# OzAmram/CaloDiffusion

Measured on AMD Instinct MI355X. Metric: sampled showers/sec (Dataset-2, 400-step DDIM), higher is better.
Workload: dtype f32 (convs: fp32 operands as 2-term fp16 splits on the fp16 MFMA pipe, fp32 accumulate; attention/norms fp32)

## Files before the change

calodiffusion_amd/csrc/kernels_conv_transpose.hip:

```cpp
#include "conv_internal.h"
#include <algorithm>
#include <vector>

namespace cd {

static constexpr int LDS_VOX_PAD = 4;

struct ConvTArgs {
  const float* in;
  int cin;
  const float* wpk;
  const float* bias;
  float* out;
  int Din, Hin, Win, Do, Ho, Wo;
  int KZ, SZ;
  int cout, CTtot;
  int TZ, TH, nTZ, nTH;
  int Cw;
  int CS;
  const u32x4* wpk16;
  int* status;
  const unsigned* in_absmax;
  int tr_off = 0;
};

template <int CT>
__global__ void __launch_bounds__(256) conv_transpose_kernel(ConvTArgs a) {
  extern __shared__ __attribute__((aligned(16))) float lds[];
  const int tid = threadIdx.x, lane = tid & 63, wave = tid >> 6, nw = blockDim.x >> 6;
  int bid = blockIdx.x;
  const int thi = bid % a.nTH;
  bid /= a.nTH;
  const int tzi = bid % a.nTZ;
  const int b = bid / a.nTZ;
  const int a0 = tzi * a.TZ, b0 = thi * a.TH;
  const int PZ = a.TZ + 2, PH = a.TH + 2;
  const int tileVox = PZ * PH * a.Win;
  const int ZERO = tileVox * a.CS;
  const int half = lane >> 5, col = lane & 31;
  for (int i = tid; i < a.CS; i += blockDim.x) lds[ZERO + i] = 0.f;

  {
    const int c4 = a.cin >> 2;
    const int items = tileVox * c4;
    const float* src = a.in + (size_t)b * a.Din * a.Hin * a.Win * a.cin;
    for (int idx = tid; idx < items; idx += blockDim.x) {
      const int q = idx % c4, vox = idx / c4;
      const int iw = vox % a.Win;
      const int r = vox / a.Win;
      const int lh = r % PH, lz = r / PH;
      const int gz = a0 - 1 + lz;
      int gh = (b0 - 1 + lh) % a.Hin;
      if (gh < 0) gh += a.Hin;
      f32x4 val = {0.f, 0.f, 0.f, 0.f};
      if (gz >= 0 && gz < a.Din) val = *(const f32x4*)(src + ((size_t)(gz * a.Hin + gh) * a.Win + iw) * a.cin + q * 4);
      *(f32x4*)(lds + vox * a.CS + q * 4) = val;
    }
  }
  __syncthreads();

  const int ncls = a.SZ * 4;
  const int njt = (a.TZ * a.TH * a.Cw + 31) / 32;
  const int nchunk = a.cin >> 5;
  const int T = a.KZ * 16;
  float* outb = a.out + (size_t)b * a.Do * a.Ho * a.Wo * a.cout;

  for (int job = wave; job < ncls * njt; job += nw) {
    const int cls = job / njt, jt = job % njt;
    const int pz = cls >> 2, ph = (cls >> 1) & 1, pw = cls & 1;
    const int v = jt * 32 + col;
    const int c = v % a.Cw;
    const int t = v / a.Cw;
    const int bb = t % a.TH, aa = t / a.TH;
    const int oz = a.SZ * (a0 + aa) + pz, oh = 2 * (b0 + bb) + ph, ow = 2 * c + pw;
    const bool valid = (aa < a.TZ) && (oz < a.Do) && (oh < a.Ho) && (ow < a.Wo);
    if (!__any(valid)) continue;
    const int ooff = valid ? ((oz * a.Ho + oh) * a.Wo + ow) * a.cout : -1;

    f32x16 acc[CT];
#pragma unroll
    for (int ct = 0; ct < CT; ++ct)
#pragma unroll
      for (int r = 0; r < 16; ++r) acc[ct][r] = 0.f;

    for (int kz = (pz + 1) % a.SZ; kz < a.KZ; kz += a.SZ) {
      const int lz = aa + (pz + 1 - kz) / a.SZ + 1;
      for (int kh = (ph + 3) & 1; kh < 4; kh += 2) {
        const int lh = bb + (ph + 3 - kh) / 2;
        for (int kw = (pw + 1) & 1; kw < 4; kw += 2) {
          const int iw = c + (pw + 1 - kw) / 2;
          const bool ok = valid && iw >= 0 && iw < a.Win;
          const int off = ok ? ((lz * PH + lh) * a.Win + iw) * a.CS + half * 16 : ZERO + half * 16;
          const int tap = (kz * 4 + kh) * 4 + kw;
          for (int chunk = 0; chunk < nchunk; ++chunk) {
            f32x4 av[4];
#pragma unroll
            for (int q = 0; q < 4; ++q) av[q] = *(const f32x4*)(lds + off + chunk * 32 + q * 4);
            const f32x4* wq = (const f32x4*)a.wpk + ((size_t)(chunk * T + tap) * a.CTtot) * 256 + lane;
#pragma unroll
            for (int ct = 0; ct < CT; ++ct) {
              f32x4 bw[4];
#pragma unroll
              for (int q = 0; q < 4; ++q) bw[q] = wq[ct * 256 + q * 64];
#pragma unroll
              for (int q = 0; q < 4; ++q)
#pragma unroll
                for (int e = 0; e < 4; ++e) acc[ct] = MFMA32(av[q][e], bw[q][e], acc[ct]);
            }
          }
        }
      }
    }
#pragma unroll
    for (int r = 0; r < 16; ++r) {
      const int row = (r & 3) + 8 * (r >> 2) + 4 * half;
      const int off = __shfl(ooff, row, 64);
      if (off >= 0) {
#pragma unroll
        for (int ct = 0; ct < CT; ++ct) {
          const int co = ct * 32 + col;
          outb[off + co] = acc[ct][r] + (a.bias ? a.bias[co] : 0.f);
        }
      }
    }
  }
}

template <int CT>
__global__ void __launch_bounds__(256) conv_transpose_f16x2_kernel(ConvTArgs a) {
  extern __shared__ __attribute__((aligned(16))) float lds[];
  const int tid = threadIdx.x, lane = tid & 63, wave = tid >> 6, nw = blockDim.x >> 6;
  int bid = blockIdx.x;
  const int thi = bid % a.nTH;
  bid /= a.nTH;
  const int tzi = bid % a.nTZ;
  const int b = bid / a.nTZ;
  const int a0 = tzi * a.TZ, b0 = thi * a.TH;
  const int PZ = a.TZ + 2, PH = a.TH + 2;
  const int tileVox = PZ * PH * a.Win;
  const int ZERO = tileVox * a.CS;
  const int half = lane >> 5, col = lane & 31;
  for (int i = tid; i < a.CS; i += blockDim.x) lds[ZERO + i] = 0.f;

  float gscale = 1.f, ginv = 1.f;
  if (a.in_absmax) pow2_scale_for(*a.in_absmax, &gscale, &ginv);
  {
    const int c4 = a.cin >> 2;
    const float* src = a.in + (size_t)b * a.Din * a.Hin * a.Win * a.cin;
    float amax = 0.f;
    auto stage = [&](int vox, int q, int iw, int lh, int lz) {
      const int gz = a0 - 1 + lz;
      int gh = b0 - 1 + lh;
      gh = gh < 0 ? gh + a.Hin : gh;
      gh = gh >= a.Hin ? gh - a.Hin : gh;
      gh = gh >= a.Hin ? gh - a.Hin : gh;
      f32x4 val = {0.f, 0.f, 0.f, 0.f};
      if (gz >= 0 && gz < a.Din) val = *(const f32x4*)(src + ((size_t)(gz * a.Hin + gh) * a.Win + iw) * a.cin + q * 4);
      val *= gscale;
      amax = fmaxf(amax, fmaxf(fmaxf(fabsf(val[0]), fabsf(val[1])), fmaxf(fabsf(val[2]), fabsf(val[3]))));
      u32x2 t1, t2;
      split2(val, t1, t2);
      char* dst = (char*)(lds + vox * a.CS) + (q >> 2) * 64 + (q & 3) * 8;
      *(u32x2*)dst = t1;
      *(u32x2*)(dst + 32) = t2;
    };
    const int nthr = blockDim.x;
    if (nthr % c4 == 0) {
      const int q = tid % c4, vstep = nthr / c4;
      int vox = tid / c4;
      int iw = vox % a.Win, r = vox / a.Win;
      int lh = r % PH, lz = r / PH;
      const int dw = vstep % a.Win, dr = vstep / a.Win, dh = dr % PH, dz = dr / PH;
      for (; vox < tileVox; vox += vstep) {
        stage(vox, q, iw, lh, lz);
        iw += dw; lh += dh; lz += dz;
        if (iw >= a.Win) { iw -= a.Win; lh += 1; }
        if (lh >= PH) { lh -= PH; lz += 1; }
      }
    } else {
      const int items = tileVox * c4;
      for (int idx = tid; idx < items; idx += nthr) {
        const int q = idx % c4, vox = idx / c4;
        const int iw = vox % a.Win;
        const int r = vox / a.Win;
        stage(vox, q, iw, r % PH, r / PH);
      }
    }
    if (a.status && amax > 65504.f) atomicOr(a.status, 1);
  }
  __syncthreads();

  const int szs = a.SZ - 1;
  const int ncls = a.SZ * 4;
  const int njt = (a.TZ * a.TH * a.Cw + 31) / 32;
  const int nks = a.cin >> 4;
  const int T = a.KZ * 16;
  float* outb = a.out + (size_t)b * a.Do * a.Ho * a.Wo * a.cout;

  const bool tile_major = njt >= nw;
  for (int item = wave; item < (tile_major ? njt : ncls * njt); item += nw) {
    const int jt = tile_major ? item : item % njt;
    const int v = jt * 32 + col;
    const int c = v % a.Cw;
    const int t = v / a.Cw;
    const int bb = t % a.TH, aa = t / a.TH;
  for (int ci = 0; ci < (tile_major ? ncls : 1); ++ci) {
    const int cls = tile_major ? ci : item / njt;
    const int pz = cls >> 2, ph = (cls >> 1) & 1, pw = cls & 1;
    const int oz = ((a0 + aa) << szs) + pz, oh = 2 * (b0 + bb) + ph, ow = 2 * c + pw;
    const bool valid = (aa < a.TZ) && (oz < a.Do) && (oh < a.Ho) && (ow < a.Wo);
    if (!__any(valid)) continue;
    const int ooff = valid ? ((oz * a.Ho + oh) * a.Wo + ow) * a.cout : -1;

    f32x16 accA[CT], accB[CT];
#pragma unroll
    for (int ct = 0; ct < CT; ++ct)
#pragma unroll
      for (int r = 0; r < 16; ++r) { accA[ct][r] = 0.f; accB[ct][r] = 0.f; }

    const int kz0 = (pz + 1) & szs, kh0 = (ph + 3) & 1, kw0 = (pw + 1) & 1;
    const int nkz = (a.KZ - kz0 + a.SZ - 1) >> szs;
    const int nstage = nkz * 4 * nks;
    struct Stage {
      u32x4 x1, x2, w[CT][2];
    };
    int ti_n = 0, ks_n = 0, tap_n = 0;
    const char* rec_n = nullptr;
    auto setup = [&](int ti) {
      const int kz = kz0 + ((ti >> 2) << szs), kh = kh0 + ((ti >> 1) & 1) * 2, kw = kw0 + (ti & 1) * 2;
      const int lz = aa + ((pz + 1 - kz) >> szs) + 1;
      const int lh = bb + ((ph + 3 - kh) >> 1);
      const int iw = c + ((pw + 1 - kw) >> 1);
      const bool ok = valid && iw >= 0 && iw < a.Win;
      rec_n = (const char*)(lds + (ok ? ((lz * PH + lh) * a.Win + iw) * a.CS : ZERO)) + half * 16;
      tap_n = (kz * 4 + kh) * 4 + kw;
    };
    setup(0);
    auto fetch = [&](Stage& st) {
      st.x1 = *(const u32x4*)(rec_n + ks_n * 64);
      st.x2 = *(const u32x4*)(rec_n + ks_n * 64 + 32);
      const u32x4* wq = a.wpk16 + ((size_t)(ks_n * T + tap_n) * a.CTtot) * 128 + lane;
#pragma unroll
      for (int ct = 0; ct < CT; ++ct) {
        st.w[ct][0] = wq[ct * 128];
        st.w[ct][1] = wq[ct * 128 + 64];
      }
      if (ks_n + 1 < nks) ++ks_n;
      else if (ti_n + 1 < nkz * 4) { ks_n = 0; setup(++ti_n); }
    };
    auto mfmas = [&](const Stage& st) {
#pragma unroll
      for (int ct = 0; ct < CT; ++ct) {
        accA[ct] = MFMA_F16(st.x1, st.w[ct][0], accA[ct]);
        accB[ct] = MFMA_F16(st.x1, st.w[ct][1], accB[ct]);
        accB[ct] = MFMA_F16(st.x2, st.w[ct][0], accB[ct]);
      }
    };
    Stage s0, s1, s2, s3;
    fetch(s0);
    fetch(s1);
    fetch(s2);
    for (int j = 0; j < nstage; j += 4) {
      fetch(s3);
      __builtin_amdgcn_sched_barrier(0);
      mfmas(s0);
      __builtin_amdgcn_sched_barrier(0);
      fetch(s0);
      __builtin_amdgcn_sched_barrier(0);
      if (j + 1 < nstage) mfmas(s1);
      __builtin_amdgcn_sched_barrier(0);
      fetch(s1);
      __builtin_amdgcn_sched_barrier(0);
      if (j + 2 < nstage) mfmas(s2);
      __builtin_amdgcn_sched_barrier(0);
      fetch(s2);
      __builtin_amdgcn_sched_barrier(0);
      if (j + 3 < nstage) mfmas(s3);
    }
    float* tr = lds + a.tr_off + wave * (32 * 36);
#pragma unroll
    for (int ct = 0; ct < CT; ++ct) {
      const float bv = a.bias ? a.bias[ct * 32 + col] : 0.f;
#pragma unroll
      for (int r = 0; r < 16; ++r)
        tr[((r & 3) + 8 * (r >> 2) + 4 * half) * 36 + col] = (accA[ct][r] + accB[ct][r] * (1.f / 2048.f)) * ginv + bv;
      asm volatile("s_waitcnt lgkmcnt(0)" ::: "memory");
#pragma unroll
      for (int k = 0; k < 4; ++k) {
        const int row = 8 * k + (lane >> 3);
        const int off = __shfl(ooff, row, 64);
        const f32x4 q = *(const f32x4*)(tr + row * 36 + (lane & 7) * 4);
        if (off >= 0) *(f32x4*)(outb + off + ct * 32 + (lane & 7) * 4) = q;
      }
      asm volatile("s_waitcnt lgkmcnt(0)" ::: "memory");
    }
  }
  }
}

template <int CT>
static void launch_convT_inst(const ConvTArgs& a, dim3 grid, size_t lds, hipStream_t s) {
  static bool attr_set = false;
  if (!attr_set) {
    CD_HIP(hipFuncSetAttribute((const void*)conv_transpose_kernel<CT>, hipFuncAttributeMaxDynamicSharedMemorySize, 160 * 1024));
    CD_HIP(hipFuncSetAttribute((const void*)conv_transpose_f16x2_kernel<CT>, hipFuncAttributeMaxDynamicSharedMemorySize, 160 * 1024));
    attr_set = true;
  }
  if (a.wpk16) hipLaunchKernelGGL((conv_transpose_f16x2_kernel<CT>), grid, dim3(256), lds, s, a);
  else hipLaunchKernelGGL((conv_transpose_kernel<CT>), grid, dim3(256), lds, s, a);
  CD_HIP(hipGetLastError());
}

void launch_conv_transpose_mfma(const float* in, int cin, const float* wpk, const float* bias, float* out, int batch,
                                int cout, Dims3 din, Dims3 dout, int kz, int sz, hipStream_t s, const void* wpk_f16x2,
                                int* status, const unsigned* in_absmax) {
  CD_REQUIRE(cin % 32 == 0 && cout % 32 == 0, "conv_transpose: channels must be multiples of 32");
  CD_REQUIRE(sz == 1 || sz == 2, "conv_transpose: z stride must be 1 or 2");
  const bool full_range = conv_precision() != PREC_F16X2;
  ConvTArgs a;
  a.wpk16 = full_range ? nullptr : (const u32x4*)wpk_f16x2;
  a.status = status;
  a.in_absmax = in_absmax;
  a.in = in; a.cin = cin; a.wpk = wpk; a.bias = bias; a.out = out;
  a.Din = din.d; a.Hin = din.h; a.Win = din.w; a.Do = dout.d; a.Ho = dout.h; a.Wo = dout.w;
  a.KZ = kz; a.SZ = sz; a.cout = cout; a.CTtot = cout / 32;
  a.Cw = (dout.w + 1) / 2;
  a.CS = cin + LDS_VOX_PAD;
  const int Az = (dout.d + sz - 1) / sz, Bh = (dout.h + 1) / 2;
  struct TT { int tz, th; double score; };
  std::vector<TT> all;
  for (int TZ = 1; TZ <= Az; ++TZ)
    for (int TH = 1; TH <= Bh; ++TH) {
      const size_t lds = ((size_t)(TZ + 2) * (TH + 2) * din.w + 1) * a.CS * 4;
      if (lds > 140 * 1024) break;
      if (TH != Bh && (Bh + TH - 1) / TH == (Bh + TH) / (TH + 1)) continue;
      if (TZ != Az && (Az + TZ - 1) / TZ == (Az + TZ) / (TZ + 1)) continue;
      const long nblocks = (long)batch * ((Az + TZ - 1) / TZ) * ((Bh + TH - 1) / TH);
      const double ratio = (double)TZ * TH / ((double)(TZ + 2) * (TH + 2));
      const double fill = nblocks >= 512 ? 1.0 : (double)nblocks / 512.0;
      all.push_back({TZ, TH, ratio * fill});
    }
  CD_REQUIRE(!all.empty(), "conv_transpose: no tile fits in LDS");
  std::stable_sort(all.begin(), all.end(), [](const TT& x, const TT& y) { return x.score > y.score; });
  std::vector<TT> cand;
  for (size_t i = 0; i < all.size() && cand.size() < 8; ++i) cand.push_back(all[i]);
  for (size_t i = 8; i < all.size() && cand.size() < 14; i += (all.size() - 8) / 6 + 1) cand.push_back(all[i]);
  char cat[128];
  std::snprintf(cat, sizeof cat, "convT%dx4x4 C%d->%d @%dx%dx%d", kz, cin, cout, din.d, din.h, din.w);
  prof::Scope scope(cat, s, 2.0 * kz * 16 * cin * cout * (double)din.vox() * batch,
                    4.0 * batch * ((double)din.vox() * cin + (double)dout.vox() * cout));
  auto launch = [&](const TT& t) {
    ConvTArgs b = a;
    b.TZ = t.tz; b.TH = t.th;
    b.nTZ = (Az + b.TZ - 1) / b.TZ; b.nTH = (Bh + b.TH - 1) / b.TH;
    size_t lds = ((size_t)(b.TZ + 2) * (b.TH + 2) * din.w + 1) * b.CS * 4;
    if (b.wpk16) {
      lds = (lds + 15) & ~(size_t)15;
      b.tr_off = (int)(lds / 4);
      lds += 4 * 32 * 36 * 4;
    }
    dim3 grid((unsigned)(batch * b.nTZ * b.nTH));
    switch (b.CTtot) {
      case 1: launch_convT_inst<1>(b, grid, lds, s); break;
      case 2: launch_convT_inst<2>(b, grid, lds, s); break;
      case 3: launch_convT_inst<3>(b, grid, lds, s); break;
      case 4: launch_convT_inst<4>(b, grid, lds, s); break;
      default: CD_REQUIRE(false, "conv_transpose: more than 128 output channels unsupported");
    }
  };
  char key[192];
  std::snprintf(key, sizeof key, "%s k%d s%d b%d%s", cat, kz, sz, batch, a.wpk16 ? " f16x2" : "");
  const int pick = autotune(key, (int)cand.size(), [&](int i) { launch(cand[i]); }, s);
  launch(cand[pick < 0 ? 0 : pick]);
}

}
```

Measured before the change: 90.89.

## Add weight-resident transposed-conv kernel with software-pipelined LDS loads

Adds a weight-resident variant of the f16x2 transposed-conv kernel for cin==cout in {32,64}. Each wave keeps one output class/channel-tile's weights in registers and sweeps all spatial tiles, prefetching LDS fragments three steps ahead and overlapping the previous tile's epilogue with the current MFMAs. The input staging loop is also unrolled so several global loads are in flight at once. Autotune candidates now include resident tile shapes with their own scoring, and env overrides are added. The cost is much higher register pressure, which may lower occupancy.

After: 91.11 (median of 2 runs). About the same (+0.2%).

```diff
diff --git a/calodiffusion_amd/csrc/kernels_conv_transpose.hip b/calodiffusion_amd/csrc/kernels_conv_transpose.hip
--- a/calodiffusion_amd/csrc/kernels_conv_transpose.hip
+++ b/calodiffusion_amd/csrc/kernels_conv_transpose.hip
@@ -1,5 +1,6 @@
 #include "conv_internal.h"
 #include <algorithm>
+#include <cstring>
 #include <vector>
 
 namespace cd {
@@ -24,6 +25,129 @@
   int tr_off = 0;
 };
 
+template <int NTAP, int NKS>
+__device__ __forceinline__ void convt_resident_job(const ConvTArgs& a, const float* lds, float* tr, float* outb, int cls, int ct, int a0,
+                                                   int b0, int PH, int ZERO, int njt, float ginv, int lane) {
+  constexpr int NST = NTAP * NKS, PF = 3;
+  static_assert(NST > PF, "convt_resident_job: pipeline deeper than the job");
+  const int half = lane >> 5, col = lane & 31;
+  const int szs = a.SZ - 1;
+  const int pz = cls >> 2, ph = (cls >> 1) & 1, pw = cls & 1;
+  const int kz0 = (pz + 1) & szs, kh0 = (ph + 3) & 1, kw0 = (pw + 1) & 1;
+  const int T = a.KZ * 16;
+  u32x4 w[NST][2];
+  int dB[NTAP];
+#pragma unroll
+  for (int ti = 0; ti < NTAP; ++ti) {
+    const int kz = kz0 + ((ti >> 2) << szs), kh = kh0 + ((ti >> 1) & 1) * 2, kw = kw0 + (ti & 1) * 2;
+    const int tap = (kz * 4 + kh) * 4 + kw;
+    dB[ti] = (((((pz + 1 - kz) >> szs) * PH + ((ph + 3 - kh) >> 1)) * a.Win + ((pw + 1 - kw) >> 1)) * a.CS) * 4;
+#pragma unroll
+    for (int ks = 0; ks < NKS; ++ks) {
+      const u32x4* wq = a.wpk16 + ((size_t)(ks * T + tap) * a.CTtot + ct) * 128 + lane;
+      w[ti * NKS + ks][0] = wq[0];
+      w[ti * NKS + ks][1] = wq[64];
+    }
+  }
+  const int dw0 = (pw + 1 - kw0) >> 1;
+  const int zaddr = ZERO * 4 + half * 16;
+  const float bv = a.bias ? a.bias[ct * 32 + col] : 0.f;
+
+  int c = col % a.Cw, bb, aa;
+  {
+    const int t = col / a.Cw;
+    bb = t % a.TH;
+    aa = t / a.TH;
+  }
+  const int dc = 32 % a.Cw, dt = 32 / a.Cw, db = dt % a.TH, da = dt / a.TH;
+  struct Frag {
+    u32x4 x1, x2;
+  };
+  bool valid = false, ok0 = false, ok1 = false;
+  int ooff = -1, base = 0;
+  auto place = [&]() {
+    const int oz = ((a0 + aa) << szs) + pz, oh = 2 * (b0 + bb) + ph, ow = 2 * c + pw;
+    valid = (aa < a.TZ) && (oz < a.Do) && (oh < a.Ho) && (ow < a.Wo);
+    ooff = valid ? ((oz * a.Ho + oh) * a.Wo + ow) * a.cout : -1;
+    base = ((((aa + 1) * PH + bb) * a.Win + c) * a.CS) * 4 + half * 16;
+    const int iw0 = c + dw0;
+    ok0 = valid && iw0 >= 0 && iw0 < a.Win;
+    ok1 = valid && iw0 >= 1 && iw0 - 1 < a.Win;
+  };
+  auto load = [&](Frag& f, int j) {
+    const int ti = j / NKS, ks = j % NKS;
+    const char* rec = (const char*)lds + (((ti & 1) ? ok1 : ok0) ? base + dB[ti] : zaddr);
+    f.x1 = *(const u32x4*)(rec + ks * 64);
+    f.x2 = *(const u32x4*)(rec + ks * 64 + 32);
+  };
+  Frag pre[PF];
+  place();
+#pragma unroll
+  for (int j = 0; j < PF; ++j) load(pre[j], j);
+  int ooff_prev = -1;
+  auto epi_write = [&](const f32x16& pA, const f32x16& pB) {
+#pragma unroll
+    for (int r = 0; r < 16; ++r)
+      tr[((r & 3) + 8 * (r >> 2) + 4 * half) * 36 + col] = (pA[r] + pB[r] * (1.f / 2048.f)) * ginv + bv;
+  };
+  f32x4 oq[4];
+  int ooffq[4];
+  auto epi_read = [&]() {
+#pragma unroll
+    for (int k = 0; k < 4; ++k) {
+      const int row = 8 * k + (lane >> 3);
+      ooffq[k] = __shfl(ooff_prev, row, 64);
+      oq[k] = *(const f32x4*)(tr + row * 36 + (lane & 7) * 4);
+    }
+  };
+  auto epi_store = [&]() {
+#pragma unroll
+    for (int k = 0; k < 4; ++k)
+      if (ooffq[k] >= 0) *(f32x4*)(outb + ooffq[k] + ct * 32 + (lane & 7) * 4) = oq[k];
+  };
+  auto tile = [&](f32x16& accA, f32x16& accB, const f32x16& pA, const f32x16& pB) {
+#pragma unroll
+    for (int r = 0; r < 16; ++r) { accA[r] = 0.f; accB[r] = 0.f; }
+    Frag x[NST];
+#pragma unroll
+    for (int j = 0; j < PF; ++j) x[j] = pre[j];
+#pragma unroll
+    for (int j = 0; j < NST; ++j) {
+      if (j + PF < NST) load(x[j + PF], j + PF);
+      accA = MFMA_F16(x[j].x1, w[j][0], accA);
+      accB = MFMA_F16(x[j].x1, w[j][1], accB);
+      accB = MFMA_F16(x[j].x2, w[j][0], accB);
+      if (j == 0) epi_write(pA, pB);
+      if (j == 2) epi_read();
+      if (j == 5) epi_store();
+    }
+    ooff_prev = ooff;
+    c += dc; bb += db; aa += da;
+    if (c >= a.Cw) { c -= a.Cw; bb += 1; }
+    if (bb >= a.TH) { bb -= a.TH; aa += 1; }
+    place();
+#pragma unroll
+    for (int j = 0; j < PF; ++j) load(pre[j], j);
+  };
+  f32x16 a0A, a0B, a1A, a1B;
+#pragma unroll
+  for (int r = 0; r < 16; ++r) { a1A[r] = 0.f; a1B[r] = 0.f; }
+  int jt = 0;
+  for (; jt + 1 < njt; jt += 2) {
+    tile(a0A, a0B, a1A, a1B);
+    tile(a1A, a1B, a0A, a0B);
+  }
+  if (jt < njt) {
+    tile(a0A, a0B, a1A, a1B);
+    epi_write(a0A, a0B);
+  } else {
+    epi_write(a1A, a1B);
+  }
+  epi_read();
+  epi_store();
+  asm volatile("s_waitcnt lgkmcnt(0)" ::: "memory");
+}
+
 template <int CT>
 __global__ void __launch_bounds__(256) conv_transpose_kernel(ConvTArgs a) {
   extern __shared__ __attribute__((aligned(16))) float lds[];
@@ -126,7 +250,7 @@
   }
 }
 
-template <int CT>
+template <int CT, bool RES = false>
 __global__ void __launch_bounds__(256) conv_transpose_f16x2_kernel(ConvTArgs a) {
   extern __shared__ __attribute__((aligned(16))) float lds[];
   const int tid = threadIdx.x, lane = tid & 63, wave = tid >> 6, nw = blockDim.x >> 6;
@@ -148,14 +272,15 @@
     const int c4 = a.cin >> 2;
     const float* src = a.in + (size_t)b * a.Din * a.Hin * a.Win * a.cin;
     float amax = 0.f;
-    auto stage = [&](int vox, int q, int iw, int lh, int lz) {
+    auto src_off = [&](int iw, int lh, int lz) {
       const int gz = a0 - 1 + lz;
       int gh = b0 - 1 + lh;
       gh = gh < 0 ? gh + a.Hin : gh;
       gh = gh >= a.Hin ? gh - a.Hin : gh;
       gh = gh >= a.Hin ? gh - a.Hin : gh;
-      f32x4 val = {0.f, 0.f, 0.f, 0.f};
-      if (gz >= 0 && gz < a.Din) val = *(const f32x4*)(src + ((size_t)(gz * a.Hin + gh) * a.Win + iw) * a.cin + q * 4);
+      return (gz >= 0 && gz < a.Din) ? (long)((size_t)(gz * a.Hin + gh) * a.Win + iw) * a.cin : -1L;
+    };
+    auto put = [&](int vox, int q, f32x4 val) {
       val *= gscale;
       amax = fmaxf(amax, fmaxf(fmaxf(fabsf(val[0]), fabsf(val[1])), fmaxf(fabsf(val[2]), fabsf(val[3]))));
       u32x2 t1, t2;
@@ -166,16 +291,27 @@
     };
     const int nthr = blockDim.x;
     if (nthr % c4 == 0) {
+      constexpr int U = RES ? 8 : 4;
       const int q = tid % c4, vstep = nthr / c4;
       int vox = tid / c4;
       int iw = vox % a.Win, r = vox / a.Win;
       int lh = r % PH, lz = r / PH;
       const int dw = vstep % a.Win, dr = vstep / a.Win, dh = dr % PH, dz = dr / PH;
-      for (; vox < tileVox; vox += vstep) {
-        stage(vox, q, iw, lh, lz);
-        iw += dw; lh += dh; lz += dz;
-        if (iw >= a.Win) { iw -= a.Win; lh += 1; }
-        if (lh >= PH) { lh -= PH; lz += 1; }
+      while (vox < tileVox) {
+        f32x4 val[U];
+        bool in[U];
+#pragma unroll
+        for (int u = 0; u < U; ++u) {
+          const long off = src_off(iw, lh, lz);
+          in[u] = off >= 0 && vox + u * vstep < tileVox;
+          val[u] = *(const f32x4*)(src + (in[u] ? off : 0) + q * 4);
+          iw += dw; lh += dh; lz += dz;
+          if (iw >= a.Win) { iw -= a.Win; lh += 1; }
+          if (lh >= PH) { lh -= PH; lz += 1; }
+        }
+#pragma unroll
+        for (int u = 0; u < U; ++u, vox += vstep)
+          if (vox < tileVox) put(vox, q, in[u] ? val[u] : f32x4{0.f, 0.f, 0.f, 0.f});
       }
     } else {
       const int items = tileVox * c4;
@@ -183,7 +319,10 @@
         const int q = idx % c4, vox = idx / c4;
         const int iw = vox % a.Win;
         const int r = vox / a.Win;
-        stage(vox, q, iw, r % PH, r / PH);
+        const long off = src_off(iw, r % PH, r / PH);
+        f32x4 val = {0.f, 0.f, 0.f, 0.f};
+        if (off >= 0) val = *(const f32x4*)(src + off + q * 4);
+        put(vox, q, val);
       }
     }
     if (a.status && amax > 65504.f) atomicOr(a.status, 1);
@@ -196,6 +335,19 @@
   const int nks = a.cin >> 4;
   const int T = a.KZ * 16;
   float* outb = a.out + (size_t)b * a.Do * a.Ho * a.Wo * a.cout;
+
+  if constexpr (RES) {
+    constexpr int NKS = 2 * CT;
+    float* tr = lds + a.tr_off + wave * (32 * 36);
+    for (int job = wave; job < ncls * CT; job += nw) {
+      const int cls = job % ncls, ct = job / ncls;
+      const int nkz = (a.KZ - (((cls >> 2) + 1) & szs) + a.SZ - 1) >> szs;
+      if (nkz == 1) convt_resident_job<4, NKS>(a, lds, tr, outb, cls, ct, a0, b0, PH, ZERO, njt, ginv, lane);
+      else if (nkz == 2) convt_resident_job<8, NKS>(a, lds, tr, outb, cls, ct, a0, b0, PH, ZERO, njt, ginv, lane);
+      else if constexpr (CT == 1) convt_resident_job<12, NKS>(a, lds, tr, outb, cls, ct, a0, b0, PH, ZERO, njt, ginv, lane);
+    }
+    return;
+  }
 
   const bool tile_major = njt >= nw;
   for (int item = wave; item < (tile_major ? njt : ncls * njt); item += nw) {
@@ -298,15 +450,26 @@
   }
 }
 
+static bool convt_resident_ok(const ConvTArgs& a) {
+  if (!a.wpk16 || a.in_absmax || a.KZ < 1 || a.KZ > 3 || a.cin != a.cout) return false;
+  const int nkz_max = a.SZ == 1 ? a.KZ : (a.KZ + 1) / 2;
+  return (a.cin == 32 || a.cin == 64) && nkz_max * 4 * (a.cin / 16) * 8 <= 256;
+}
+
 template <int CT>
-static void launch_convT_inst(const ConvTArgs& a, dim3 grid, size_t lds, hipStream_t s) {
+static void launch_convT_inst(const ConvTArgs& a, dim3 grid, size_t lds, hipStream_t s, bool resident) {
   static bool attr_set = false;
   if (!attr_set) {
     CD_HIP(hipFuncSetAttribute((const void*)conv_transpose_kernel<CT>, hipFuncAttributeMaxDynamicSharedMemorySize, 160 * 1024));
     CD_HIP(hipFuncSetAttribute((const void*)conv_transpose_f16x2_kernel<CT>, hipFuncAttributeMaxDynamicSharedMemorySize, 160 * 1024));
+    if constexpr (CT <= 2)
+      CD_HIP(hipFuncSetAttribute((const void*)conv_transpose_f16x2_kernel<CT, true>, hipFuncAttributeMaxDynamicSharedMemorySize, 160 * 1024));
     attr_set = true;
   }
-  if (a.wpk16) hipLaunchKernelGGL((conv_transpose_f16x2_kernel<CT>), grid, dim3(256), lds, s, a);
+  if (resident) {
+    if constexpr (CT <= 2) hipLaunchKernelGGL((conv_transpose_f16x2_kernel<CT, true>), grid, dim3(256), lds, s, a);
+    else CD_REQUIRE(false, "conv_transpose: no weight-resident instance for more than 64 output channels");
+  } else if (a.wpk16) hipLaunchKernelGGL((conv_transpose_f16x2_kernel<CT>), grid, dim3(256), lds, s, a);
   else hipLaunchKernelGGL((conv_transpose_kernel<CT>), grid, dim3(256), lds, s, a);
   CD_HIP(hipGetLastError());
 }
@@ -327,28 +490,43 @@
   a.Cw = (dout.w + 1) / 2;
   a.CS = cin + LDS_VOX_PAD;
   const int Az = (dout.d + sz - 1) / sz, Bh = (dout.h + 1) / 2;
-  struct TT { int tz, th; double score; };
-  std::vector<TT> all;
+  struct TT { int tz, th; double score; bool res; };
+  const bool resident = convt_resident_ok(a) && !getenv("CD_NO_CONVT_RESIDENT");
+  int force_tz = 0, force_th = 0;
+  if (const char* e = getenv("CD_CONVT_TILE")) {
+    CD_REQUIRE(std::sscanf(e, "%d,%d", &force_tz, &force_th) == 2 && force_tz >= 1 && force_tz <= Az && force_th >= 1 && force_th <= Bh,
+               "CD_CONVT_TILE: want tz,th inside the class-index grid");
+    CD_REQUIRE(((size_t)(force_tz + 2) * (force_th + 2) * din.w + 1) * a.CS * 4 <= 140 * 1024, "CD_CONVT_TILE: the tile does not fit in LDS");
+  }
+  std::vector<TT> all, all_res;
   for (int TZ = 1; TZ <= Az; ++TZ)
     for (int TH = 1; TH <= Bh; ++TH) {
       const size_t lds = ((size_t)(TZ + 2) * (TH + 2) * din.w + 1) * a.CS * 4;
       if (lds > 140 * 1024) break;
-      if (TH != Bh && (Bh + TH - 1) / TH == (Bh + TH) / (TH + 1)) continue;
-      if (TZ != Az && (Az + TZ - 1) / TZ == (Az + TZ) / (TZ + 1)) continue;
       const long nblocks = (long)batch * ((Az + TZ - 1) / TZ) * ((Bh + TH - 1) / TH);
       const double ratio = (double)TZ * TH / ((double)(TZ + 2) * (TH + 2));
-      const double fill = nblocks >= 512 ? 1.0 : (double)nblocks / 512.0;
-      all.push_back({TZ, TH, ratio * fill});
+      if (!(TH != Bh && (Bh + TH - 1) / TH == (Bh + TH) / (TH + 1)) && !(TZ != Az && (Az + TZ - 1) / TZ == (Az + TZ) / (TZ + 1))) {
+        const double fill = nblocks >= 512 ? 1.0 : (double)nblocks / 512.0;
+        all.push_back({TZ, TH, ratio * fill, false});
+      }
+      if (resident && !(TH > 1 && (Bh + TH - 2) / (TH - 1) == (Bh + TH - 1) / TH) && !(TZ > 1 && (Az + TZ - 2) / (TZ - 1) == (Az + TZ - 1) / TZ)) {
+        const int njt = (TZ * TH * a.Cw + 31) / 32;
+        const long rounds = (nblocks + 255) / 256;
+        all_res.push_back({TZ, TH, ratio * ((double)nblocks / (rounds * 256.0)) * (njt / (njt + 1.5)), true});
+      }
     }
   CD_REQUIRE(!all.empty(), "conv_transpose: no tile fits in LDS");
-  std::stable_sort(all.begin(), all.end(), [](const TT& x, const TT& y) { return x.score > y.score; });
+  const auto by_score = [](const TT& x, const TT& y) { return x.score > y.score; };
+  std::stable_sort(all.begin(), all.end(), by_score);
+  std::stable_sort(all_res.begin(), all_res.end(), by_score);
   std::vector<TT> cand;
-  for (size_t i = 0; i < all.size() && cand.size() < 8; ++i) cand.push_back(all[i]);
-  for (size_t i = 8; i < all.size() && cand.size() < 14; i += (all.size() - 8) / 6 + 1) cand.push_back(all[i]);
+  for (size_t i = 0; i < all_res.size() && i < 8; ++i) cand.push_back(all_res[i]);
+  const size_t nres = cand.size();
+  for (size_t i = 0; i < all.size() && cand.size() < nres + 8; ++i) cand.push_back(all[i]);
+  for (size_t i = 8; i < all.size() && cand.size() < nres + 14; i += (all.size() - 8) / 6 + 1) cand.push_back(all[i]);
+  if (force_tz) cand.assign(1, TT{force_tz, force_th, 0.0, resident});
   char cat[128];
   std::snprintf(cat, sizeof cat, "convT%dx4x4 C%d->%d @%dx%dx%d", kz, cin, cout, din.d, din.h, din.w);
-  prof::Scope scope(cat, s, 2.0 * kz * 16 * cin * cout * (double)din.vox() * batch,
-                    4.0 * batch * ((double)din.vox() * cin + (double)dout.vox() * cout));
   auto launch = [&](const TT& t) {
     ConvTArgs b = a;
     b.TZ = t.tz; b.TH = t.th;
@@ -361,17 +539,21 @@
     }
     dim3 grid((unsigned)(batch * b.nTZ * b.nTH));
     switch (b.CTtot) {
-      case 1: launch_convT_inst<1>(b, grid, lds, s); break;
-      case 2: launch_convT_inst<2>(b, grid, lds, s); break;
-      case 3: launch_convT_inst<3>(b, grid, lds, s); break;
-      case 4: launch_convT_inst<4>(b, grid, lds, s); break;
+      case 1: launch_convT_inst<1>(b, grid, lds, s, t.res); break;
+      case 2: launch_convT_inst<2>(b, grid, lds, s, t.res); break;
+      case 3: launch_convT_inst<3>(b, grid, lds, s, t.res); break;
+      case 4: launch_convT_inst<4>(b, grid, lds, s, t.res); break;
       default: CD_REQUIRE(false, "conv_transpose: more than 128 output channels unsupported");
     }
   };
   char key[192];
-  std::snprintf(key, sizeof key, "%s k%d s%d b%d%s", cat, kz, sz, batch, a.wpk16 ? " f16x2" : "");
-  const int pick = autotune(key, (int)cand.size(), [&](int i) { launch(cand[i]); }, s);
-  launch(cand[pick < 0 ? 0 : pick]);
-}
-
-}
+  std::snprintf(key, sizeof key, "%s k%d s%d b%d%s%s", cat, kz, sz, batch, a.wpk16 ? " f16x2" : "", resident ? " res" : "");
+  const int pick = force_tz ? 0 : autotune(key, (int)cand.size(), [&](int i) { launch(cand[i]); }, s);
+  const TT& run = cand[pick < 0 ? 0 : pick];
+  if (run.res) std::strncat(cat, " resident", sizeof cat - std::strlen(cat) - 1);
+  prof::Scope scope(cat, s, 2.0 * kz * 16 * cin * cout * (double)din.vox() * batch,
+                    4.0 * batch * ((double)din.vox() * cin + (double)dout.vox() * cout));
+  launch(run);
+}
+
+}
```
